# gunrock/graphblast

Measured on NVIDIA H100. Metric: MTEPS, higher is better.
Workload: dtype f32

## Files before the change

### graphblast_b200/csrc/graphblas/backend/cuda/bfs_fused.hpp

```cpp
#ifndef GRAPHBLAS_BACKEND_CUDA_BFS_FUSED_HPP_
#define GRAPHBLAS_BACKEND_CUDA_BFS_FUSED_HPP_

#include "graphblas/backend/cuda/kernels/bfs_fused.cuh"

namespace graphblas {
namespace backend {

inline bool bfsFusedApplies(Descriptor* desc) {
  Desc_value mask_mode, outp, inp0, inp1;
  if (desc->get(GrB_MASK, &mask_mode) != GrB_SUCCESS) return false;
  desc->get(GrB_OUTP, &outp); desc->get(GrB_INP0, &inp0); desc->get(GrB_INP1, &inp1);
  return desc->struconly() && desc->opreuse() && desc->earlyexit() && desc->fusedmask() &&
         mask_mode == GrB_DEFAULT && outp == GrB_DEFAULT && inp0 == GrB_DEFAULT &&
         inp1 == GrB_DEFAULT && !desc->debug() && desc->timing_ != 1;
}

inline bool bfsTrace() {
  static const bool on = getEnv("GB200_BFS_TRACE", 0) != 0;
  return on;
}

struct BfsScratchLayout {
  size_t visited[2], frontier, next, counters, heavy, walk, walk_count, walk_chunks,
         level8, bytes;
};

inline BfsScratchLayout bfsScratchLayout(Index n) {
  const size_t nwords = (static_cast<size_t>(n) + 31)/32;
  const size_t nchunks = (nwords + 31)/32;
  BfsScratchLayout l;
  ScratchLayout at;
  l.visited[0]  = at.place(nwords*sizeof(unsigned int));
  l.visited[1]  = at.place(nwords*sizeof(unsigned int));
  l.frontier    = at.place(nwords*sizeof(unsigned int));
  l.next        = at.place(nwords*sizeof(unsigned int));
  l.counters    = at.place(GB_BFS_NCOUNTERS*sizeof(unsigned long long));
  l.heavy       = at.place(GB_BFS_HEAVY_CAP*sizeof(Index));
  l.walk        = at.place(nchunks*GB_BFS_CHUNK*sizeof(Index));
  l.walk_count  = at.place(nchunks*sizeof(int));
  l.walk_chunks = at.place(nchunks*sizeof(Index));
  l.level8      = at.place(static_cast<size_t>(n));
  l.bytes = at.bytes;
  return l;
}

inline void bfsFusedStats(Descriptor* desc, Index n, unsigned long long out[6]) {
  static_assert(GB_BFS_CELL_FOUND_PUSHING == GB_BFS_CELL_LEVELS + 5,
                "the six result cells are not consecutive");
  for (int i = 0; i < 6; ++i) out[i] = 0ull;
  const BfsScratchLayout l = bfsScratchLayout(n);
  const size_t cells = l.counters + GB_BFS_CELL_LEVELS*sizeof(unsigned long long);
  if (desc->scratchSize(GB_SCRATCH_BFS) < cells + 6*sizeof(unsigned long long)) return;
  unsigned char* base = reinterpret_cast<unsigned char*>(desc->scratch(GB_SCRATCH_BFS, 0));
  CUDA_CALL(cudaMemcpyAsync(out, base + cells, 6*sizeof(unsigned long long),
      cudaMemcpyDeviceToHost, gbStream()));
  runtime().sync();
}

template <typename a>
Info bfsFused(Vector<float>* v, const Matrix<a>* A, Index s, Descriptor* desc, int* depth) {
  SparseMatrix<a>* S = const_cast<SparseMatrix<a>*>(&A->sparse_);
  const Index n = S->nrows_;
  if (n != S->ncols_) return GrB_DIMENSION_MISMATCH;
  if (S->d_csrRowPtr_ == NULL || S->d_cscColPtr_ == NULL) return GrB_UNINITIALIZED_OBJECT;
  cudaStream_t stream = gbStream();
  CHECK(v->setStorage(GrB_DENSE));
  CHECK(v->dense_.allocateGpu());

  const int fw = 1;
  const Index* probe = pullMaxDegreeNeighbours(S, fw, S->d_cscColPtr_, S->d_cscRowInd_, n);

  const BfsScratchLayout l = bfsScratchLayout(n);
  unsigned char* base =
      reinterpret_cast<unsigned char*>(desc->scratch(GB_SCRATCH_BFS, l.bytes));
  BfsFusedArgs args;
  args.push_ptr = S->d_csrRowPtr_;  args.push_ind = S->d_csrColInd_;
  args.pull_ptr = S->d_cscColPtr_;  args.pull_ind = S->d_cscRowInd_;
  args.pull_probe = probe;
  args.pull_empty = pullEmptyRowBits(probe, n);
  args.push_empty = S->sameStructure() ? NULL : pullEmptyRowBits(
      pullFirstNeighbours(S, 0, S->d_csrRowPtr_, S->d_csrColInd_, n), n);
  args.n = n;
  args.source = s;
  args.max_levels = desc->max_niter_;
  args.switchpoint = desc->switchpoint();
  args.mode = desc->mxvRoute();
  args.levels = v->dense_.d_val_;
  args.visited[0]  = reinterpret_cast<unsigned int*>(base + l.visited[0]);
  args.visited[1]  = reinterpret_cast<unsigned int*>(base + l.visited[1]);
  args.frontier    = reinterpret_cast<unsigned int*>(base + l.frontier);
  args.next        = reinterpret_cast<unsigned int*>(base + l.next);
  args.counters    = reinterpret_cast<unsigned long long*>(base + l.counters);
  args.heavy       = reinterpret_cast<Index*>(base + l.heavy);
  args.walk        = reinterpret_cast<Index*>(base + l.walk);
  args.walk_count  = reinterpret_cast<int*>(base + l.walk_count);
  args.walk_chunks = reinterpret_cast<Index*>(base + l.walk_chunks);
  args.level8      = base + l.level8;

  args.trace = bfsTrace();
  args.prof_bytes = NULL;
  if (profiler().enabled) {
    profiler().ensureCells();
    args.prof_bytes = profiler().d_cells + GB_PROF_PULL_BOOL;
  }

  profiler().begin(GB_PROF_PULL_BOOL, stream);
  const Info launched = args.mode == 1
      ? launchCooperative<bfsFusedKernel<GB_BFS_PUSH_NT, GB_BFS_PUSH_MINB, false>,
                          GB_BFS_PUSH_NT>(stream, args)
      : launchCooperative<bfsFusedKernel<GB_BFS_NT, GB_BFS_MINB, true>, GB_BFS_NT>(stream, args);
  if (launched != GrB_SUCCESS) return launched;
  profiler().end(GB_PROF_PULL_BOOL, stream, 0.0);
  v->dense_.touched();
  if (args.trace) {
    unsigned long long cells[GB_BFS_NCOUNTERS];
    CUDA_CALL(cudaMemcpyAsync(cells, args.counters, sizeof(cells), cudaMemcpyDeviceToHost,
        stream));
    runtime().sync();
    const unsigned long long* const clock = cells + GB_BFS_CELL_LEVEL_CLOCK;
    const int levels = static_cast<int>(
        cells[GB_BFS_CELL_LEVELS] < GB_BFS_TIMED_LEVELS - 1 ? cells[GB_BFS_CELL_LEVELS]
                                                            : GB_BFS_TIMED_LEVELS - 1);
    fprintf(stderr, "bfs trace: set-up %.1fus",
            1e-3*static_cast<double>((clock[0] >> 1) - cells[GB_BFS_CELL_START_CLOCK]));
    for (int l = 1; l <= levels; ++l) {
      const unsigned long long start = clock[l - 1] >> 1, end = clock[l] >> 1;
      const unsigned long long scan = cells[GB_BFS_CELL_SCAN_CLOCK + l];
      if (clock[l] & 1ull)
        fprintf(stderr, " L%d pull %.1fus (scan %.1f walk %.1f, %llu walked, %llu listed)",
                l, 1e-3*static_cast<double>(end - start),
                1e-3*static_cast<double>(scan - start),
                1e-3*static_cast<double>(end - scan), cells[GB_BFS_CELL_WALKED + l],
                cells[GB_BFS_CELL_LISTED_CHUNKS + l]);
      else
        fprintf(stderr, " L%d push %.1fus", l, 1e-3*static_cast<double>(end - start));
    }
    fprintf(stderr, " end-pass %.1fus\n",
            1e-3*static_cast<double>(cells[GB_BFS_CELL_END_PASS_CLOCK] -
                                     cells[GB_BFS_CELL_LAST_LEVEL_CLOCK]));
  }
  if (depth != NULL) {
    const unsigned long long levels = runtime().fetch(args.counters + GB_BFS_CELL_LEVELS);
    *depth = static_cast<int>(levels);
    desc->lastmxv_ = GrB_PULLONLY;
  }
  return GrB_SUCCESS;
}

}
}

#endif
```

### graphblast_b200/csrc/graphblas/backend/cuda/kernels/bfs_fused.cuh

```cuda
#ifndef GRAPHBLAS_BACKEND_CUDA_KERNELS_BFS_FUSED_CUH_
#define GRAPHBLAS_BACKEND_CUDA_KERNELS_BFS_FUSED_CUH_

#include <cooperative_groups.h>

#include "graphblas/backend/cuda/kernels/common.cuh"

namespace graphblas {
namespace backend {

#ifndef GB_BFS_NT
#define GB_BFS_NT     512
#endif
#ifndef GB_BFS_MINB
#define GB_BFS_MINB   2
#endif
#ifndef GB_BFS_PUSH_NT
#define GB_BFS_PUSH_NT   768
#endif
#ifndef GB_BFS_PUSH_MINB
#define GB_BFS_PUSH_MINB 2
#endif
#ifndef GB_BFS_BATCH
#define GB_BFS_BATCH  4
#endif
#ifndef GB_BFS_WALK_STEP
#define GB_BFS_WALK_STEP 4
#endif
#ifndef GB_BFS_WALK_WARP
#define GB_BFS_WALK_WARP 32
#endif
#ifndef GB_BFS_WALK_INLINE
#define GB_BFS_WALK_INLINE 64
#endif
#define GB_BFS_HEAVY  2048
#define GB_BFS_HEAVY_CAP 4096
#define GB_BFS_CHUNK  1024

struct BfsFusedArgs {
  const Index* push_ptr;   const Index* push_ind;
  const Index* pull_ptr;   const Index* pull_ind;
  const Index* pull_probe;
  const unsigned int* pull_empty;
  const unsigned int* push_empty;
  int   trace;
  unsigned long long* prof_bytes;
  Index n;
  Index source;
  int   max_levels;
  float switchpoint;
  int   mode;
  float*        levels;
  unsigned char* level8;
  unsigned int* visited[2];
  unsigned int* frontier;
  unsigned int* next;
  unsigned long long* counters;
  Index*        heavy;
  Index*        walk;
  int*          walk_count;
  Index*        walk_chunks;
};

#define GB_BFS_TIMED_LEVELS 16

enum BfsCell {
  GB_BFS_CELL_FOUND = 0,
  GB_BFS_CELL_HEAVY = GB_BFS_CELL_FOUND + 3,
  GB_BFS_CELL_LEVELS = GB_BFS_CELL_HEAVY + 3,
  GB_BFS_CELL_INSPECTED,
  GB_BFS_CELL_PULL_LEVELS,
  GB_BFS_CELL_PUSHED_VERTICES,
  GB_BFS_CELL_PUSHED_EDGES,
  GB_BFS_CELL_FOUND_PUSHING,
  GB_BFS_CELL_LEVEL_CLOCK,
  GB_BFS_CELL_START_CLOCK = GB_BFS_CELL_LEVEL_CLOCK + GB_BFS_TIMED_LEVELS,
  GB_BFS_CELL_END_PASS_CLOCK,
  GB_BFS_CELL_LAST_LEVEL_CLOCK,
  GB_BFS_CELL_WALK_CLAIM = 35,
  GB_BFS_CELL_LISTED = GB_BFS_CELL_WALK_CLAIM + 3,
  GB_BFS_CELL_SCAN_CLOCK = 44,
  GB_BFS_CELL_WALKED = GB_BFS_CELL_SCAN_CLOCK + GB_BFS_TIMED_LEVELS,
  GB_BFS_CELL_LISTED_CHUNKS = GB_BFS_CELL_WALKED + GB_BFS_TIMED_LEVELS,
  GB_BFS_NCOUNTERS = 128
};
static_assert(GB_BFS_CELL_LISTED_CHUNKS + GB_BFS_TIMED_LEVELS <= GB_BFS_NCOUNTERS,
              "the per-level cells of the last timed level are past the counters");

__device__ __forceinline__ unsigned long long* bfsLevelCell(unsigned long long* cells,
                                                            int first, int level) {
  return cells + first + level % 3;
}
__device__ __forceinline__ void bfsZeroNextCell(unsigned long long* cells, int first,
                                                int level) {
  cells[first + (level + 1) % 3] = 0ull;
}

__device__ __forceinline__ unsigned long long bfsClockNs() {
  unsigned long long t;
  asm volatile("mov.u64 %0, %globaltimer;" : "=l"(t));
  return t;
}

template <typename V>
__device__ __forceinline__ bool bfsClaim(unsigned int* visited, V vtx) {
  const unsigned int bit = 1u << (vtx & 31);
  unsigned int* word = visited + (vtx >> 5);
  if (*reinterpret_cast<volatile unsigned int*>(word) & bit) return false;
  return (atomicOr(word, bit) & bit) == 0;
}

__device__ __forceinline__ void bfsSetLevel(const BfsFusedArgs& a, Index row, int lv) {
  if (lv < 255) {
    a.level8[row] = static_cast<unsigned char>(lv);
  } else {
    a.level8[row] = 255;
    a.levels[row] = static_cast<float>(lv);
  }
}

__device__ __forceinline__ Index bfsClaimChunk(unsigned long long* cell, int lane) {
  unsigned long long c = 0ull;
  if (lane == 0) c = atomicAdd(cell, 1ull);
  return static_cast<Index>(__shfl_sync(GB_FULL_MASK, c, 0));
}

__device__ __forceinline__ unsigned int* bfsVis(const BfsFusedArgs& a, int vsel) {
  return vsel ? a.visited[1] : a.visited[0];
}
__device__ __forceinline__ unsigned int* bfsVisOther(const BfsFusedArgs& a, int vsel) {
  return vsel ? a.visited[0] : a.visited[1];
}
__device__ __forceinline__ unsigned int* bfsF(const BfsFusedArgs& a, int fsel) {
  return fsel ? a.next : a.frontier;
}
__device__ __forceinline__ unsigned int* bfsN(const BfsFusedArgs& a, int fsel) {
  return fsel ? a.frontier : a.next;
}

__device__ __forceinline__ unsigned int bfsIsolated(const BfsFusedArgs& a, Index w) {
  return a.pull_empty[w] & (a.push_empty != NULL ? a.push_empty[w] : 0xffffffffu);
}

__device__ __forceinline__ bool bfsWalkRows(const BfsFusedArgs& a, int vsel, Index row,
                                            bool active, int lane, int& inspected) {
  Index k = 0, end = 0;
  if (active) {
    k = __ldg(a.pull_ptr + row);
    end = __ldg(a.pull_ptr + row + 1);
  }
  const Index stop = (end - k > GB_BFS_WALK_WARP + GB_BFS_WALK_STEP)
                     ? k + GB_BFS_WALK_STEP : end;
  bool found = false;
  while (k < stop && !found) {
    Index col[GB_BFS_WALK_STEP];
    unsigned int wv[GB_BFS_WALK_STEP];
#pragma unroll
    for (int u = 0; u < GB_BFS_WALK_STEP; ++u)
      col[u] = (k + u < stop) ? __ldg(a.pull_ind + k + u) : static_cast<Index>(-1);
#pragma unroll
    for (int u = 0; u < GB_BFS_WALK_STEP; ++u)
      wv[u] = (col[u] >= 0) ? bfsVis(a, vsel)[col[u] >> 5] : 0u;
#pragma unroll
    for (int u = 0; u < GB_BFS_WALK_STEP; ++u) {
      if (found || col[u] < 0) continue;
      ++inspected;
      found = (wv[u] >> (col[u] & 31)) & 1u;
    }
    k += GB_BFS_WALK_STEP;
  }
  unsigned int longs = __ballot_sync(GB_FULL_MASK, !found && k < end);
  while (longs != 0u) {
    const int src = __ffs(longs) - 1;
    longs &= longs - 1u;
    const Index lend = __shfl_sync(GB_FULL_MASK, end, src);
    bool hit = false;
    for (Index lk = __shfl_sync(GB_FULL_MASK, k, src); lk < lend && !hit; lk += 32) {
      bool v = false;
      if (lk + lane < lend) {
        const Index col = __ldg(a.pull_ind + lk + lane);
        v = (bfsVis(a, vsel)[col >> 5] >> (col & 31)) & 1u;
      }
      const unsigned int b = __ballot_sync(GB_FULL_MASK, v);
      hit = (b != 0u);
      if (lane == 0)
        inspected += hit ? __ffs(b) : (lend - lk < 32 ? lend - lk : 32);
    }
    if (lane == src) found = hit;
  }
  return found;
}

template <int NT, int MINB, bool PULL>
__global__ void __launch_bounds__(NT, MINB)
bfsFusedKernel(BfsFusedArgs a) {
  namespace cg = cooperative_groups;
  cg::grid_group grid = cg::this_grid();
  __shared__ int s_red[NT/32];
  __shared__ unsigned int s_found[PULL ? NT/32 : 1][PULL ? 32 : 1];

  const Index n = a.n;
  const Index nwords = (n + 31) >> 5;
  const int lane = threadIdx.x & 31;
  const Index gtid = blockIdx.x*NT + threadIdx.x;
  const Index gthreads = gridDim.x*NT;
  const Index gwarp = gtid >> 5;
  const Index gwarps = gthreads >> 5;
  const Index nchunks = (nwords + 31) >> 5;

  if (gtid == 0) a.counters[GB_BFS_CELL_START_CLOCK] = bfsClockNs();
  if (gtid == 0) a.level8[a.source] = 1;
  for (Index w = gtid; w < nwords; w += gthreads) {
    const unsigned int seed = (w == (a.source >> 5)) ? (1u << (a.source & 31)) : 0u;
    a.visited[0][w] = seed | bfsIsolated(a, w);
    a.visited[1][w] = 0u; a.frontier[w] = seed; a.next[w] = 0u;
  }
  if (gtid <= GB_BFS_CELL_FOUND_PUSHING) a.counters[gtid] = 0ull;
  if (gtid >= GB_BFS_CELL_WALK_CLAIM && gtid < GB_BFS_CELL_LISTED + 3) a.counters[gtid] = 0ull;
  if (gtid >= GB_BFS_CELL_WALKED && gtid < GB_BFS_CELL_WALKED + GB_BFS_TIMED_LEVELS)
    a.counters[gtid] = 0ull;
  grid.sync();
  if (gtid == 0) a.counters[GB_BFS_CELL_LEVEL_CLOCK] = bfsClockNs() << 1;

  int vsel = 0;
  int fsel = 0;
  unsigned int fcount = 1u;
  bool dense = PULL && (a.mode == 2);
  float prev_ratio = 0.f;
  int inspected = 0;
  int pushed_vertices = 0;
  unsigned int pushed_edges = 0u;
  int pull_levels = 0;
  int level = 1;

  for (; level <= a.max_levels && fcount > 0u; ++level) {
    if (PULL && a.mode == 0) {
      const float ratio = static_cast<float>(fcount)/static_cast<float>(n);
      if (!dense) {
        if (ratio > a.switchpoint && ratio > prev_ratio) dense = true; else prev_ratio = ratio;
      } else {
        if (ratio <= a.switchpoint && ratio < prev_ratio) dense = false; else prev_ratio = ratio;
      }
    }
    unsigned long long* const count_cell = bfsLevelCell(a.counters, GB_BFS_CELL_FOUND, level);
    unsigned long long* const heavy_cell = bfsLevelCell(a.counters, GB_BFS_CELL_HEAVY, level);
    if (gtid == 0) {
      bfsZeroNextCell(a.counters, GB_BFS_CELL_FOUND, level);
      bfsZeroNextCell(a.counters, GB_BFS_CELL_HEAVY, level);
      bfsZeroNextCell(a.counters, GB_BFS_CELL_WALK_CLAIM, level);
      bfsZeroNextCell(a.counters, GB_BFS_CELL_LISTED, level);
    }
    int found_here = 0;

    if (!dense) {
      for (Index w0 = gwarp*32; w0 < nwords; w0 += gwarps*32) {
        const Index mine = w0 + lane;
        unsigned int my_bits = (mine < nwords) ? bfsF(a, fsel)[mine] : 0u;
        if (my_bits != 0u) bfsF(a, fsel)[mine] = 0u;
        unsigned int pending = __ballot_sync(GB_FULL_MASK, my_bits != 0u);
        while (pending != 0u) {
          const int src_lane = __ffs(pending) - 1;
          pending &= pending - 1u;
          unsigned int bits = __shfl_sync(GB_FULL_MASK, my_bits, src_lane);
          const Index w = w0 + src_lane;
          while (bits != 0u) {
            const int b = __ffs(bits) - 1;
            bits &= bits - 1u;
            const Index u = w*32 + b;
            const Index beg = __ldg(a.push_ptr + u);
            const Index deg = __ldg(a.push_ptr + u + 1) - beg;
            if (lane == 0) { ++pushed_vertices; pushed_edges += deg; }
            if (deg > GB_BFS_HEAVY) {
              unsigned long long slot = 0ull;
              if (lane == 0) slot = atomicAdd(heavy_cell, 1ull);
              slot = __shfl_sync(GB_FULL_MASK, slot, 0);
              if (slot < GB_BFS_HEAVY_CAP) {
                if (lane == 0) a.heavy[slot] = u;
                continue;
              }
            }
            for (Index k = lane; k < deg; k += 32) {
              const Index nbr = __ldg(a.push_ind + beg + k);
              if (bfsClaim(bfsVis(a, vsel), nbr)) {
                bfsSetLevel(a, nbr, level + 1);
                atomicOr(bfsN(a, fsel) + (nbr >> 5), 1u << (nbr & 31));
                ++found_here;
              }
            }
          }
        }
      }
      grid.sync();
      const unsigned long long listed =
          *reinterpret_cast<volatile unsigned long long*>(heavy_cell);
      const int nheavy = (listed > GB_BFS_HEAVY_CAP) ? GB_BFS_HEAVY_CAP
                                                     : static_cast<int>(listed);
      if (nheavy > 0) {
        for (int h = 0; h < nheavy; ++h) {
          const Index u = a.heavy[h];
          const Index beg = __ldg(a.push_ptr + u);
          const Index deg = __ldg(a.push_ptr + u + 1) - beg;
          for (Index k = gtid; k < deg; k += gthreads) {
            const Index nbr = __ldg(a.push_ind + beg + k);
            if (bfsClaim(bfsVis(a, vsel), nbr)) {
              bfsSetLevel(a, nbr, level + 1);
              atomicOr(bfsN(a, fsel) + (nbr >> 5), 1u << (nbr & 31));
              ++found_here;
            }
          }
        }
      }
    } else if (PULL) {
      ++pull_levels;
      unsigned long long* const walk_cell =
          bfsLevelCell(a.counters, GB_BFS_CELL_WALK_CLAIM, level);
      unsigned long long* const list_cell = bfsLevelCell(a.counters, GB_BFS_CELL_LISTED, level);
      Index c = gwarp;
      unsigned int next_vis = (c < nchunks && c*32 + lane < nwords)
                              ? bfsVis(a, vsel)[c*32 + lane] : 0xffffffffu;
      while (c < nchunks) {
        const Index word = c*32 + lane;
        const unsigned int my_vis = next_vis;
        const Index c_next = c + gwarps;
        next_vis = (c_next < nchunks && c_next*32 + lane < nwords)
                   ? bfsVis(a, vsel)[c_next*32 + lane] : 0xffffffffu;
        Index* const walk = a.walk + c*GB_BFS_CHUNK;
        int nwalk = 0;
        unsigned int my_out = 0u;
        unsigned int open = __ballot_sync(GB_FULL_MASK, my_vis != 0xffffffffu);
        unsigned int my_open = ~my_vis;
        if (word == nwords - 1 && (n & 31) != 0) my_open &= (1u << (n & 31)) - 1u;
        const int nopen = __popc(my_open);
        int first = nopen;
#pragma unroll
        for (int off = 1; off < 32; off <<= 1) {
          const int t = __shfl_up_sync(GB_FULL_MASK, first, off);
          if (lane >= off) first += t;
        }
        const int total = __shfl_sync(GB_FULL_MASK, first, 31);
        first -= nopen;
        const int word_batches = (__popc(open) + GB_BFS_BATCH - 1)/GB_BFS_BATCH;
        const int row_batches = (total + 32*GB_BFS_BATCH - 1)/(32*GB_BFS_BATCH);
        if (2*row_batches < word_batches) {
          open = 0u;
          unsigned int* const found_bits = s_found[threadIdx.x >> 5];
          found_bits[lane] = 0u;
          __syncwarp();
          for (int r0 = 0; r0 < total; r0 += 32*GB_BFS_BATCH) {
            int local[GB_BFS_BATCH];
            Index f[GB_BFS_BATCH];
#pragma unroll
            for (int j = 0; j < GB_BFS_BATCH; ++j) {
              const int r = r0 + 32*j + lane;
              int wl = 0, base = 0;
#pragma unroll
              for (int step = 16; step > 0; step >>= 1) {
                const int fs = __shfl_sync(GB_FULL_MASK, first, wl + step);
                if (fs <= r) { wl += step; base = fs; }
              }
              unsigned int m = __shfl_sync(GB_FULL_MASK, my_open, wl);
              int k = r - base, b = 0;
#pragma unroll
              for (int width = 16; width > 0; width >>= 1) {
                const int lo = __popc(m & ((1u << width) - 1u));
                if (k >= lo) { k -= lo; b += width; m >>= width; }
              }
              local[j] = wl*32 + b;
              f[j] = (r < total) ? ldStream32(a.pull_probe + c*GB_BFS_CHUNK + local[j])
                                 : static_cast<Index>(-1);
            }
            unsigned int pword[GB_BFS_BATCH];
#pragma unroll
            for (int j = 0; j < GB_BFS_BATCH; ++j)
              pword[j] = (f[j] != static_cast<Index>(-1))
                         ? bfsVis(a, vsel)[(f[j] & 0x7fffffff) >> 5] : 0u;
#pragma unroll
            for (int j = 0; j < GB_BFS_BATCH; ++j) {
              if (r0 + 32*j >= total) break;
              const bool found = (pword[j] >> (f[j] & 31)) & 1u;
              inspected += (f[j] != static_cast<Index>(-1)) ? 1 : 0;
              const bool walk_row = f[j] >= 0 && !found;
              const Index row = c*GB_BFS_CHUNK + local[j];
              const unsigned int walkers = __ballot_sync(GB_FULL_MASK, walk_row);
              if (walk_row) walk[nwalk + __popc(walkers & ((1u << lane) - 1u))] = row;
              nwalk += __popc(walkers);
              if (found) {
                atomicOr(found_bits + (local[j] >> 5), 1u << (local[j] & 31));
                bfsSetLevel(a, row, level + 1);
                ++found_here;
              }
            }
          }
          __syncwarp();
          my_out = found_bits[lane];
        }
        while (open != 0u) {
          const unsigned int batch = open;
          Index f[GB_BFS_BATCH];
#pragma unroll
          for (int j = 0; j < GB_BFS_BATCH; ++j) {
            const int wl = __ffs(open) - 1;
            open &= open - 1u;
            f[j] = static_cast<Index>(-1);
            if (wl >= 0) {
              const unsigned int m = __shfl_sync(GB_FULL_MASK, my_vis, wl);
              const Index row = c*GB_BFS_CHUNK + wl*32 + lane;
              if (row < n && !((m >> lane) & 1u)) f[j] = ldStream32(a.pull_probe + row);
            }
          }
          unsigned int pword[GB_BFS_BATCH];
#pragma unroll
          for (int j = 0; j < GB_BFS_BATCH; ++j)
            pword[j] = (f[j] != static_cast<Index>(-1))
                       ? bfsVis(a, vsel)[(f[j] & 0x7fffffff) >> 5] : 0u;
          unsigned int hit = 0u, more = 0u;
#pragma unroll
          for (int j = 0; j < GB_BFS_BATCH; ++j) {
            const bool found = (pword[j] >> (f[j] & 31)) & 1u;
            inspected += (f[j] != static_cast<Index>(-1)) ? 1 : 0;
            hit |= static_cast<unsigned int>(found) << j;
            more |= static_cast<unsigned int>(f[j] >= 0 && !found) << j;
          }
          unsigned int rest = batch;
#pragma unroll
          for (int j = 0; j < GB_BFS_BATCH && rest != 0u; ++j) {
            const int wl = __ffs(rest) - 1;
            rest &= rest - 1u;
            const Index row = c*GB_BFS_CHUNK + wl*32 + lane;
            const bool found = (hit >> j) & 1u, walk_row = (more >> j) & 1u;
            const unsigned int walkers = __ballot_sync(GB_FULL_MASK, walk_row);
            if (walk_row) walk[nwalk + __popc(walkers & ((1u << lane) - 1u))] = row;
            nwalk += __popc(walkers);
            const unsigned int out = __ballot_sync(GB_FULL_MASK, found);
            if (found) { bfsSetLevel(a, row, level + 1); ++found_here; }
            if (lane == wl) my_out = out;
          }
        }
        if (nwalk > 0 && nwalk <= GB_BFS_WALK_INLINE) {
          unsigned int* const found_bits = s_found[threadIdx.x >> 5];
          found_bits[lane] = my_out;
          __syncwarp();
          for (int i0 = 0; i0 < nwalk; i0 += 32) {
            const bool active = i0 + lane < nwalk;
            const Index row = active ? walk[i0 + lane] : 0;
            if (bfsWalkRows(a, vsel, row, active, lane, inspected)) {
              const int local = row & (GB_BFS_CHUNK - 1);
              atomicOr(found_bits + (local >> 5), 1u << (local & 31));
              bfsSetLevel(a, row, level + 1);
              ++found_here;
            }
          }
          __syncwarp();
          my_out = found_bits[lane];
        }
        if (word < nwords) {
          bfsN(a, fsel)[word] = my_out;
          bfsVisOther(a, vsel)[word] = my_vis | my_out;
          bfsF(a, fsel)[word] = 0u;
        }
        if (lane == 0 && nwalk > 0) {
          if (nwalk > GB_BFS_WALK_INLINE) {
            a.walk_count[c] = nwalk;
            a.walk_chunks[atomicAdd(list_cell, 1ull)] = c;
          }
          if (a.trace && level < GB_BFS_TIMED_LEVELS)
            atomicAdd(a.counters + GB_BFS_CELL_WALKED + level,
                      static_cast<unsigned long long>(nwalk));
        }
        c = c_next;
      }
      grid.sync();
      const Index nlisted = static_cast<Index>(
          *reinterpret_cast<volatile unsigned long long*>(list_cell));
      if (gtid == 0 && level < GB_BFS_TIMED_LEVELS) {
        a.counters[GB_BFS_CELL_SCAN_CLOCK + level] = bfsClockNs();
        if (a.trace)
          a.counters[GB_BFS_CELL_LISTED_CHUNKS + level] = static_cast<unsigned long long>(nlisted);
      }
      for (Index i = gwarp; i < nlisted; ) {
        const Index i_next = gwarps + bfsClaimChunk(walk_cell, lane);
        const Index c = a.walk_chunks[i];
        const int nwalk = a.walk_count[c];
        for (int i0 = 0; i0 < nwalk; i0 += 32) {
          const bool active = i0 + lane < nwalk;
          const Index row = active ? a.walk[c*GB_BFS_CHUNK + i0 + lane] : 0;
          if (bfsWalkRows(a, vsel, row, active, lane, inspected)) {
            const unsigned int bit = 1u << (row & 31);
            atomicOr(bfsN(a, fsel) + (row >> 5), bit);
            atomicOr(bfsVisOther(a, vsel) + (row >> 5), bit);
            bfsSetLevel(a, row, level + 1);
            ++found_here;
          }
        }
        i = i_next;
      }
    }
    const int block_found = blockSum<NT>(found_here, s_red);
    if (threadIdx.x == 0 && block_found) {
      atomicAdd(count_cell, static_cast<unsigned long long>(block_found));
      if (!dense)
        atomicAdd(a.counters + GB_BFS_CELL_FOUND_PUSHING,
                  static_cast<unsigned long long>(block_found));
    }
    grid.sync();
    if (gtid == 0 && level < GB_BFS_TIMED_LEVELS)
      a.counters[GB_BFS_CELL_LEVEL_CLOCK + level] = (bfsClockNs() << 1) | (dense ? 1ull : 0ull);
    fcount = static_cast<unsigned int>(
        *reinterpret_cast<volatile unsigned long long*>(count_cell));
    if (dense) vsel ^= 1;
    fsel ^= 1;
  }
  if (gtid == 0) a.counters[GB_BFS_CELL_LAST_LEVEL_CLOCK] = bfsClockNs();
  const unsigned int* const cut_rows = (fcount > 0u) ? bfsF(a, fsel) : NULL;
  const bool lines = (reinterpret_cast<uintptr_t>(a.levels) & 15u) == 0u;
  const Index nblocks = (nwords + 15) >> 4;
  if (PULL) {
    auto load_block = [&](Index blk, unsigned int& reached, unsigned int (&b)[4]) {
      reached = 0u;
#pragma unroll
      for (int j = 0; j < 4; ++j) b[j] = 0u;
      if (blk >= nblocks) return;
      const Index w = blk*16 + (lane & 15);
      if (lane < 16 && w < nwords) {
        reached = bfsVis(a, vsel)[w] & ~bfsIsolated(a, w);
        if (cut_rows != NULL) reached &= ~cut_rows[w];
        if (w == (a.source >> 5)) reached |= 1u << (a.source & 31);
      }
#pragma unroll
      for (int j = 0; j < 4; ++j) {
        const Index row = blk*512 + 128*j + 4*lane;
        if (lines && row + 4 <= n) b[j] = *reinterpret_cast<const unsigned int*>(a.level8 + row);
      }
    };
    unsigned int next_reached, next_b[4];
    load_block(gwarp, next_reached, next_b);
    for (Index blk = gwarp; blk < nblocks; blk += gwarps) {
      const Index r0 = blk*512;
      const unsigned int reached = next_reached;
      unsigned int lb[4];
#pragma unroll
      for (int j = 0; j < 4; ++j) lb[j] = next_b[j];
      load_block(blk + gwarps, next_reached, next_b);
#pragma unroll
      for (int j = 0; j < 4; ++j) {
        const unsigned int bits =
            (__shfl_sync(GB_FULL_MASK, reached, 4*j + (lane >> 3)) >> (4*(lane & 7))) & 0xfu;
        const Index row = r0 + 128*j + 4*lane;
        if (row >= n) continue;
        if (lines && row + 4 <= n) {
          const unsigned int b = lb[j];
          float f[4];
          bool escape = false;
#pragma unroll
          for (int k = 0; k < 4; ++k) {
            const unsigned int byte = (b >> (8*k)) & 0xffu;
            const bool r = (bits >> k) & 1u;
            escape |= r && byte == 255u;
            f[k] = r ? static_cast<float>(byte) : 0.f;
          }
          if (!escape) {
            __stcs(reinterpret_cast<float4*>(a.levels + row), make_float4(f[0], f[1], f[2], f[3]));
            continue;
          }
        }
        for (int k = 0; k < 4 && row + k < n; ++k) {
          if (!((bits >> k) & 1u)) {
            a.levels[row + k] = 0.f;
          } else {
            const unsigned int byte = a.level8[row + k];
            if (byte != 255u) a.levels[row + k] = static_cast<float>(byte);
          }
        }
      }
    }
  } else {
    for (Index blk = gwarp; blk < nblocks; blk += gwarps) {
      const Index r0 = blk*512;
      const Index w = blk*16 + (lane & 15);
      unsigned int reached = 0u;
      if (lane < 16 && w < nwords) {
        reached = bfsVis(a, vsel)[w] & ~bfsIsolated(a, w);
        if (cut_rows != NULL) reached &= ~cut_rows[w];
        if (w == (a.source >> 5)) reached |= 1u << (a.source & 31);
      }
#pragma unroll
      for (int j = 0; j < 4; ++j) {
        const unsigned int bits =
            (__shfl_sync(GB_FULL_MASK, reached, 4*j + (lane >> 3)) >> (4*(lane & 7))) & 0xfu;
        const Index row = r0 + 128*j + 4*lane;
        if (row >= n) continue;
        if (lines && row + 4 <= n) {
          const unsigned int b = *reinterpret_cast<const unsigned int*>(a.level8 + row);
          float f[4];
          bool escape = false;
#pragma unroll
          for (int k = 0; k < 4; ++k) {
            const unsigned int byte = (b >> (8*k)) & 0xffu;
            const bool r = (bits >> k) & 1u;
            escape |= r && byte == 255u;
            f[k] = r ? static_cast<float>(byte) : 0.f;
          }
          if (!escape) {
            __stcs(reinterpret_cast<float4*>(a.levels + row), make_float4(f[0], f[1], f[2], f[3]));
            continue;
          }
        }
        for (int k = 0; k < 4 && row + k < n; ++k) {
          if (!((bits >> k) & 1u)) {
            a.levels[row + k] = 0.f;
          } else {
            const unsigned int byte = a.level8[row + k];
            if (byte != 255u) a.levels[row + k] = static_cast<float>(byte);
          }
        }
      }
    }
  }
  if (a.trace) {
    grid.sync();
    if (gtid == 0) a.counters[GB_BFS_CELL_END_PASS_CLOCK] = bfsClockNs();
  }
  const int block_insp = blockSum<NT>(inspected, s_red);
  const int block_pv = blockSum<NT>(pushed_vertices, s_red);
  if (threadIdx.x == 0) {
    if (block_insp)
      atomicAdd(a.counters + GB_BFS_CELL_INSPECTED, static_cast<unsigned long long>(block_insp));
    if (block_pv)
      atomicAdd(a.counters + GB_BFS_CELL_PUSHED_VERTICES,
                static_cast<unsigned long long>(block_pv));
  }
  if (pushed_edges)
    atomicAdd(a.counters + GB_BFS_CELL_PUSHED_EDGES,
              static_cast<unsigned long long>(pushed_edges));
  if (gtid == 0) {
    a.counters[GB_BFS_CELL_LEVELS] = static_cast<unsigned long long>(level - 1);
    a.counters[GB_BFS_CELL_PULL_LEVELS] = static_cast<unsigned long long>(pull_levels);
  }
  if (a.prof_bytes != NULL) {
    if (pushed_edges) atomicAdd(a.prof_bytes, 8ull*pushed_edges);
    if (threadIdx.x == 0) {
      unsigned long long bytes = 4ull*static_cast<unsigned long long>(block_insp) +
                                 12ull*static_cast<unsigned long long>(block_pv);
      if (blockIdx.x == 0)
        bytes += static_cast<unsigned long long>(pull_levels)*
                     (12ull*static_cast<unsigned long long>(n) + 4ull) +
                 8ull*(*reinterpret_cast<volatile unsigned long long*>(
                           a.counters + GB_BFS_CELL_FOUND_PUSHING));
      if (bytes) atomicAdd(a.prof_bytes, bytes);
    }
  }
}

}
}

#endif
```

Before: 2.452 million.

## Skip second grid barrier when no heavy or walk work is listed; expand source directly

Restructures each BFS level so the second-phase work (heavy push vertices or listed pull walk chunks) runs only when the listed count is nonzero. Otherwise the level ends after a single grid.sync instead of two. Level 1 expands the source vertex across the whole grid directly instead of scanning the frontier bitmap, and init no longer clears visited[1] or seeds the frontier. Found-count accumulation is moved into each phase, and the trace clock encoding gains a bit for phase count. The risk is correctness: the visited[1] init removal and the changed reduction ordering must stay consistent.

```diff
diff --git a/graphblast_b200/csrc/graphblas/backend/cuda/bfs_fused.hpp b/graphblast_b200/csrc/graphblas/backend/cuda/bfs_fused.hpp
--- a/graphblast_b200/csrc/graphblas/backend/cuda/bfs_fused.hpp
+++ b/graphblast_b200/csrc/graphblas/backend/cuda/bfs_fused.hpp
@@ -122,10 +122,12 @@
         cells[GB_BFS_CELL_LEVELS] < GB_BFS_TIMED_LEVELS - 1 ? cells[GB_BFS_CELL_LEVELS]
                                                             : GB_BFS_TIMED_LEVELS - 1);
     fprintf(stderr, "bfs trace: set-up %.1fus",
-            1e-3*static_cast<double>((clock[0] >> 1) - cells[GB_BFS_CELL_START_CLOCK]));
+            1e-3*static_cast<double>((clock[0] >> 2) - cells[GB_BFS_CELL_START_CLOCK]));
+    int second_phases = 0;
     for (int l = 1; l <= levels; ++l) {
-      const unsigned long long start = clock[l - 1] >> 1, end = clock[l] >> 1;
+      const unsigned long long start = clock[l - 1] >> 2, end = clock[l] >> 2;
       const unsigned long long scan = cells[GB_BFS_CELL_SCAN_CLOCK + l];
+      second_phases += static_cast<int>((clock[l] >> 1) & 1ull);
       if (clock[l] & 1ull)
         fprintf(stderr, " L%d pull %.1fus (scan %.1f walk %.1f, %llu walked, %llu listed)",
                 l, 1e-3*static_cast<double>(end - start),
@@ -138,6 +140,10 @@
     fprintf(stderr, " end-pass %.1fus\n",
             1e-3*static_cast<double>(cells[GB_BFS_CELL_END_PASS_CLOCK] -
                                      cells[GB_BFS_CELL_LAST_LEVEL_CLOCK]));
+    fprintf(stderr, "bfs barriers: %llu (second phases %d%s)\n",
+            1ull + cells[GB_BFS_CELL_LEVELS] + second_phases, second_phases,
+            cells[GB_BFS_CELL_LEVELS] > static_cast<unsigned long long>(levels)
+                ? ", later levels not traced" : "");
   }
   if (depth != NULL) {
     const unsigned long long levels = runtime().fetch(args.counters + GB_BFS_CELL_LEVELS);
diff --git a/graphblast_b200/csrc/graphblas/backend/cuda/kernels/bfs_fused.cuh b/graphblast_b200/csrc/graphblas/backend/cuda/kernels/bfs_fused.cuh
--- a/graphblast_b200/csrc/graphblas/backend/cuda/kernels/bfs_fused.cuh
+++ b/graphblast_b200/csrc/graphblas/backend/cuda/kernels/bfs_fused.cuh
@@ -141,6 +141,35 @@
   return a.pull_empty[w] & (a.push_empty != NULL ? a.push_empty[w] : 0xffffffffu);
 }
 
+template <int NT>
+__device__ __forceinline__ void bfsAddFound(const BfsFusedArgs& a,
+                                            unsigned long long* count_cell, int found_here,
+                                            bool pushing, int* s_red) {
+  const int block_found = blockSum<NT>(found_here, s_red);
+  if (threadIdx.x == 0 && block_found) {
+    atomicAdd(count_cell, static_cast<unsigned long long>(block_found));
+    if (pushing)
+      atomicAdd(a.counters + GB_BFS_CELL_FOUND_PUSHING,
+                static_cast<unsigned long long>(block_found));
+  }
+}
+
+__device__ __forceinline__ Index bfsExpandGrid(const BfsFusedArgs& a, int vsel, int fsel,
+                                               int level, Index u, Index gtid,
+                                               Index gthreads, int& found_here) {
+  const Index beg = __ldg(a.push_ptr + u);
+  const Index deg = __ldg(a.push_ptr + u + 1) - beg;
+  for (Index k = gtid; k < deg; k += gthreads) {
+    const Index nbr = __ldg(a.push_ind + beg + k);
+    if (bfsClaim(bfsVis(a, vsel), nbr)) {
+      bfsSetLevel(a, nbr, level + 1);
+      atomicOr(bfsN(a, fsel) + (nbr >> 5), 1u << (nbr & 31));
+      ++found_here;
+    }
+  }
+  return deg;
+}
+
 __device__ __forceinline__ bool bfsWalkRows(const BfsFusedArgs& a, int vsel, Index row,
                                             bool active, int lane, int& inspected) {
   Index k = 0, end = 0;
@@ -212,14 +241,14 @@
   for (Index w = gtid; w < nwords; w += gthreads) {
     const unsigned int seed = (w == (a.source >> 5)) ? (1u << (a.source & 31)) : 0u;
     a.visited[0][w] = seed | bfsIsolated(a, w);
-    a.visited[1][w] = 0u; a.frontier[w] = seed; a.next[w] = 0u;
+    a.frontier[w] = 0u; a.next[w] = 0u;
   }
   if (gtid <= GB_BFS_CELL_FOUND_PUSHING) a.counters[gtid] = 0ull;
   if (gtid >= GB_BFS_CELL_WALK_CLAIM && gtid < GB_BFS_CELL_LISTED + 3) a.counters[gtid] = 0ull;
   if (gtid >= GB_BFS_CELL_WALKED && gtid < GB_BFS_CELL_WALKED + GB_BFS_TIMED_LEVELS)
     a.counters[gtid] = 0ull;
   grid.sync();
-  if (gtid == 0) a.counters[GB_BFS_CELL_LEVEL_CLOCK] = bfsClockNs() << 1;
+  if (gtid == 0) a.counters[GB_BFS_CELL_LEVEL_CLOCK] = bfsClockNs() << 2;
 
   int vsel = 0;
   int fsel = 0;
@@ -251,7 +280,11 @@
     }
     int found_here = 0;
 
-    if (!dense) {
+    if (!dense && level == 1) {
+      const Index deg = bfsExpandGrid(a, vsel, fsel, level, a.source, gtid, gthreads,
+                                      found_here);
+      if (gtid == 0) { ++pushed_vertices; pushed_edges += deg; }
+    } else if (!dense) {
       for (Index w0 = gwarp*32; w0 < nwords; w0 += gwarps*32) {
         const Index mine = w0 + lane;
         unsigned int my_bits = (mine < nwords) ? bfsF(a, fsel)[mine] : 0u;
@@ -289,30 +322,8 @@
           }
         }
       }
-      grid.sync();
-      const unsigned long long listed =
-          *reinterpret_cast<volatile unsigned long long*>(heavy_cell);
-      const int nheavy = (listed > GB_BFS_HEAVY_CAP) ? GB_BFS_HEAVY_CAP
-                                                     : static_cast<int>(listed);
-      if (nheavy > 0) {
-        for (int h = 0; h < nheavy; ++h) {
-          const Index u = a.heavy[h];
-          const Index beg = __ldg(a.push_ptr + u);
-          const Index deg = __ldg(a.push_ptr + u + 1) - beg;
-          for (Index k = gtid; k < deg; k += gthreads) {
-            const Index nbr = __ldg(a.push_ind + beg + k);
-            if (bfsClaim(bfsVis(a, vsel), nbr)) {
-              bfsSetLevel(a, nbr, level + 1);
-              atomicOr(bfsN(a, fsel) + (nbr >> 5), 1u << (nbr & 31));
-              ++found_here;
-            }
-          }
-        }
-      }
     } else if (PULL) {
       ++pull_levels;
-      unsigned long long* const walk_cell =
-          bfsLevelCell(a.counters, GB_BFS_CELL_WALK_CLAIM, level);
       unsigned long long* const list_cell = bfsLevelCell(a.counters, GB_BFS_CELL_LISTED, level);
       Index c = gwarp;
       unsigned int next_vis = (c < nchunks && c*32 + lane < nwords)
@@ -468,42 +479,52 @@
         }
         c = c_next;
       }
+    }
+    for (int phase = 0; ; ++phase) {
+      bfsAddFound<NT>(a, count_cell, found_here, !dense, s_red);
       grid.sync();
-      const Index nlisted = static_cast<Index>(
-          *reinterpret_cast<volatile unsigned long long*>(list_cell));
+      const unsigned long long listed = phase ? 0ull : *reinterpret_cast<volatile unsigned long long*>(
+          bfsLevelCell(a.counters, dense ? GB_BFS_CELL_LISTED : GB_BFS_CELL_HEAVY, level));
       if (gtid == 0 && level < GB_BFS_TIMED_LEVELS) {
-        a.counters[GB_BFS_CELL_SCAN_CLOCK + level] = bfsClockNs();
-        if (a.trace)
-          a.counters[GB_BFS_CELL_LISTED_CHUNKS + level] = static_cast<unsigned long long>(nlisted);
-      }
-      for (Index i = gwarp; i < nlisted; ) {
-        const Index i_next = gwarps + bfsClaimChunk(walk_cell, lane);
-        const Index c = a.walk_chunks[i];
-        const int nwalk = a.walk_count[c];
-        for (int i0 = 0; i0 < nwalk; i0 += 32) {
-          const bool active = i0 + lane < nwalk;
-          const Index row = active ? a.walk[c*GB_BFS_CHUNK + i0 + lane] : 0;
-          if (bfsWalkRows(a, vsel, row, active, lane, inspected)) {
-            const unsigned int bit = 1u << (row & 31);
-            atomicOr(bfsN(a, fsel) + (row >> 5), bit);
-            atomicOr(bfsVisOther(a, vsel) + (row >> 5), bit);
-            bfsSetLevel(a, row, level + 1);
-            ++found_here;
-          }
-        }
-        i = i_next;
-      }
-    }
-    const int block_found = blockSum<NT>(found_here, s_red);
-    if (threadIdx.x == 0 && block_found) {
-      atomicAdd(count_cell, static_cast<unsigned long long>(block_found));
-      if (!dense)
-        atomicAdd(a.counters + GB_BFS_CELL_FOUND_PUSHING,
-                  static_cast<unsigned long long>(block_found));
-    }
-    grid.sync();
-    if (gtid == 0 && level < GB_BFS_TIMED_LEVELS)
-      a.counters[GB_BFS_CELL_LEVEL_CLOCK + level] = (bfsClockNs() << 1) | (dense ? 1ull : 0ull);
+        const unsigned long long t = bfsClockNs();
+        if (dense && phase == 0) {
+          a.counters[GB_BFS_CELL_SCAN_CLOCK + level] = t;
+          if (a.trace) a.counters[GB_BFS_CELL_LISTED_CHUNKS + level] = listed;
+        }
+        if (listed == 0ull)
+          a.counters[GB_BFS_CELL_LEVEL_CLOCK + level] =
+              (t << 2) | (static_cast<unsigned long long>(phase) << 1) | (dense ? 1ull : 0ull);
+      }
+      if (listed == 0ull) break;
+      found_here = 0;
+      if (!dense) {
+        const int nheavy = (listed > GB_BFS_HEAVY_CAP) ? GB_BFS_HEAVY_CAP
+                                                       : static_cast<int>(listed);
+        for (int h = 0; h < nheavy; ++h)
+          bfsExpandGrid(a, vsel, fsel, level, a.heavy[h], gtid, gthreads, found_here);
+      } else if (PULL) {
+        unsigned long long* const walk_cell =
+            bfsLevelCell(a.counters, GB_BFS_CELL_WALK_CLAIM, level);
+        const Index nlisted = static_cast<Index>(listed);
+        for (Index i = gwarp; i < nlisted; ) {
+          const Index i_next = gwarps + bfsClaimChunk(walk_cell, lane);
+          const Index c = a.walk_chunks[i];
+          const int nwalk = a.walk_count[c];
+          for (int i0 = 0; i0 < nwalk; i0 += 32) {
+            const bool active = i0 + lane < nwalk;
+            const Index row = active ? a.walk[c*GB_BFS_CHUNK + i0 + lane] : 0;
+            if (bfsWalkRows(a, vsel, row, active, lane, inspected)) {
+              const unsigned int bit = 1u << (row & 31);
+              atomicOr(bfsN(a, fsel) + (row >> 5), bit);
+              atomicOr(bfsVisOther(a, vsel) + (row >> 5), bit);
+              bfsSetLevel(a, row, level + 1);
+              ++found_here;
+            }
+          }
+          i = i_next;
+        }
+      }
+    }
     fcount = static_cast<unsigned int>(
         *reinterpret_cast<volatile unsigned long long*>(count_cell));
     if (dense) vsel ^= 1;
```

Measured after the change: 2.587 million (median of 6 runs). 5.5% higher.
